# mit-acl/rl_collision_avoidance

Measured on AMD Instinct MI355X. Metric: agent-steps/sec (env.step) at 4 agents x 8192 worlds per GPU, higher is better.
Workload: dtype f64

## Files before the change

### rl_collision_avoidance_amd/csrc/cavoid_capi.hip

```cpp
#include <hip/hip_runtime.h>
#include <hip/hip_ext.h>

#include <cmath>
#include <cstdlib>
#include <cstring>
#include <new>

#include "cavoid.h"
#include "cavoid_host.hpp"
#include "cavoid_kernels.hpp"
#include "cavoid_launch.hpp"
#include "cavoid_crowd.hpp"

using namespace cavoid;

thread_local int g_last_hip_error = 0;

extern "C" int cavoid_abi_version(void) { return CAVOID_ABI_VERSION; }

extern "C" int cavoid_last_hip_error(void) { return g_last_hip_error; }

extern "C" const char *cavoid_strerror(int code) {
    switch (code) {
        case CAVOID_OK: return "ok";
// ... 197 lines not shown
    cold.rvo_collab = cfg->rvo_collab_coeff; cold.rvo_radius_scale = cfg->rvo_radius_scale; cold.rvo_max_dh = cfg->rvo_max_delta_heading;
    cold.gen_min_agents = cfg->gen_min_agents; cold.gen_max_agents = cfg->gen_max_agents;
    KCold *d_cold = reinterpret_cast<KCold *>(static_cast<unsigned char *>(e->slab) + o_act + kActBytes);
    if (hipMemcpy(d_cold, &cold, sizeof(cold), hipMemcpyHostToDevice) != hipSuccess) {
        g_last_hip_error = (int)hipGetLastError();
        cavoid_destroy(e);
        return CAVOID_EHIP;
    }

    KCfg &k = e->k;
    k.cold = d_cold;
    k.dt = cfg->dt;
    k.near_goal_sq = cfg->near_goal_threshold * cfg->near_goal_threshold;
    k.collision_dist = cfg->collision_dist;
    k.close_range = cfg->getting_close_range;
    k.r_goal = cfg->reward_at_goal; k.r_coll = cfg->reward_collision; k.r_close = cfg->reward_getting_close;
    k.r_step = cfg->reward_time_step; k.close_slope = cfg->close_penalty_slope;
    k.clip_lo = cfg->reward_clip_lo; k.clip_hi = cfg->reward_clip_hi;
    k.horizon = cfg->sensing_horizon;
    k.switches = (cfg->done_agents_collide ? 0u : kSwSkipDonePairs) | (cfg->sort_round_gap ? 0u : kSwExactGap) |
                 (cfg->sort_tie_lateral ? 0u : kSwIndexTie) | (cfg->wrap_closed_end ? kSwWrapClosed : 0u);
    k.gen_mode = cfg->gen_mode; k.pool_epoch = cfg->gen_pool_epoch;
    k.rvo_enabled = cfg->rvo_enabled ? 1 : 0;
    k.max_other = cfg->max_other; k.width = 6 + 7 * cfg->max_other;
    k.sort_method = cfg->sort_method; k.dynamics = cfg->dynamics; k.actions_fp32 = cfg->actions_fp32;
    k.timeout_enabled = cfg->timeout_enabled; k.num_actions = cfg->num_actions;
    k.pool_size = cfg->gen_lookahead > 0 ? (int32_t)(e->pool_size > 0x7fffffffLL ? 0x7fffffffLL : e->pool_size) : cfg->gen_pool_size;
    k.ahead = cfg->gen_lookahead;
    k.evaluate_mode = cfg->evaluate_mode ? 1 : 0;
    k.stream_obs = (double)num_worlds * cfg->max_agents * (6 + 7 * cfg->max_other) * sizeof(float) > 16.0 * 1048576.0 ? 1 : 0;
    if (const char *ov = std::getenv("CAVOID_STREAM_OBS")) k.stream_obs = std::atoi(ov) != 0;
    k.seed_lo = 0; k.seed_hi = 0;
    k.num_worlds = num_worlds; k.world_offset = world_offset;
    k.action_table = e->d_actions;

    const int N = cfg->max_agents, wpw_max = 64 / N;
    int wpw = wpw_max;
    if (const char *ov = std::getenv("CAVOID_WPW")) { int v = std::atoi(ov); if (v >= 1 && v <= wpw_max) wpw = v; }
    k.wpw = wpw;
    const int lanes = wpw * N;
    e->latency_mode = (num_worlds * cfg->max_agents <= 64 * 2048 && (cfg->gen_pool_size > 0 || cfg->gen_lookahead > 0)) ? 1 : 0;
    if (const char *ov = std::getenv("CAVOID_PREFETCH_POOL")) {
        const int v = std::atoi(ov);
        e->latency_mode = (v != 0 && (cfg->gen_pool_size > 0 || cfg->gen_lookahead > 0)) ? 1 : 0;
        e->prefetch_single = e->latency_mode;
    }
    k.prefetch_pool = e->latency_mode;
    if (const char *ov = std::getenv("CAVOID_PIPELINE")) e->pipeline = std::atoi(ov);
    if (const char *ov = std::getenv("CAVOID_QUAD")) e->quad = std::atoi(ov);
    if (const char *ov = std::getenv("CAVOID_RELAY_CONSUMERS")) {
        const int v = std::atoi(ov);
        if (v >= 1 && v <= cavoid::kRelayMaxConsumers) e->relay_consumers = v;
    }
    if (crowd_form(N)) {
        k.rvo_lds_floats = 0;
        k.park_floats = 0;
        int rows = (crowd_key_floats(N) / (k.width + 2)) & ~3;
        if (rows < 4) rows = 4;
        if (rows > lanes) rows = lanes;
        if (const char *ov = std::getenv("CAVOID_TILE_ROWS")) { int v = std::atoi(ov); if (v >= 1 && v <= lanes) rows = v; }
        k.tile_rows = rows;
        if ((size_t)(lds_floats_block() + crowd_wave_floats(N, rows, k.width + 2)) * sizeof(float) > 65536) { cavoid_destroy(e); return CAVOID_EUNSUPPORTED; }
        e->waves_per_block = 1;
        e->grid = grid_for(e, num_worlds);
        *out = e;
        return CAVOID_OK;
    }
    k.rvo_lds_floats = cfg->rvo_enabled ? 64 * 2 * (N - 1) * 4 * 2 : 0;
    k.park_floats = ((N >= kParkFromN && !cfg->rvo_enabled) ? 3 * (N - 1) * 64 : 0) + 256;
    if (k.park_floats < lds_floats_scratch()) k.park_floats = lds_floats_scratch();
    static_assert(64 * 2 * 4 * 2 * (kParkFromN - 1) >= 3 * 64 * (kParkFromN - 1) + 256, "reset / observe of an RVO env park keys, gaps and velocities in the idle ORCA scratch");
    const int row_floats = k.width + 2;
    int tile_rows = (int)(9216 / ((size_t)row_floats * sizeof(float))) & ~3;
    if (tile_rows < 4) tile_rows = 4;
    const bool one_pass_fits = (size_t)(lds_floats_block() + lds_floats_fixed(N) + k.rvo_lds_floats + lanes * row_floats + 4) * sizeof(float) <= 65536;
    if (tile_rows > lanes || (e->latency_mode && one_pass_fits)) tile_rows = lanes;
    if (const char *ov = std::getenv("CAVOID_TILE_ROWS")) { int v = std::atoi(ov); if (v >= 1 && v <= lanes) tile_rows = v; }
    auto wave_bytes = [&](int rows) {
        int tile = (rows * row_floats + 3) & ~3;
        if (tile < k.park_floats) tile = k.park_floats;
        return (size_t)(lds_floats_fixed(N) + k.rvo_lds_floats + tile) * sizeof(float);
    };
    while (tile_rows > 4 && wave_bytes(tile_rows) + lds_floats_block() * sizeof(float) > 65536) tile_rows -= 4;
    k.tile_rows = tile_rows;
    const size_t per_wave = wave_bytes(tile_rows);
    int wpb = (int)(((size_t)65536 - lds_floats_block() * sizeof(float)) / per_wave);
    if (wpb < 1) { cavoid_destroy(e); return CAVOID_EUNSUPPORTED; }
    if (wpb > 4) wpb = 4;
    if (const char *ov = std::getenv("CAVOID_WAVES_PER_BLOCK")) { int v = std::atoi(ov); if (v >= 1 && v <= wpb) wpb = v; }
    e->waves_per_block = wpb;
    e->grid = grid_for(e, num_worlds);
    *out = e;
    return CAVOID_OK;
}

extern "C" void cavoid_destroy(cavoid_env *e) {
    if (!e) return;
    if (e->ev0) (void)hipEventDestroy(e->ev0);
    if (e->ev1) (void)hipEventDestroy(e->ev1);
    if (e->slab) (void)hipFree(e->slab);
    if (e->pool_slab) (void)hipFree(e->pool_slab);
    delete e;
}

extern "C" int64_t cavoid_num_worlds(const cavoid_env *e) { return e ? e->W : 0; }
extern "C" int32_t cavoid_obs_width(const cavoid_env *e) { return e ? e->k.width : 0; }
// ... 353 lines not shown
```

### rl_collision_avoidance_amd/csrc/cavoid_launch.hpp

```cpp
#pragma once
#include <hip/hip_runtime.h>
#include <hip/hip_ext.h>

#include <type_traits>

#include "cavoid.h"
#include "cavoid_host.hpp"
#include "cavoid_kernels.hpp"

struct cavoid_env {
    int device = 0;
    int64_t W = 0, A = 0, world_offset = 0;
    cavoid_cfg cfg{};
    cavoid::KCfg k{};
    cavoid::KState st{};
    cavoid::PoolRec *pool = nullptr;
    uint32_t *pool_episode = nullptr;
    int64_t pool_size = 0;
    int ahead_R = 0;
    uint32_t *ahead_hi[2] = {nullptr, nullptr};
    int ahead_cur = 0;
    int ahead_budget = 0;
    bool ahead_primed = false;
    bool ahead_always = false;
    int64_t ahead_refills = 0;
    int relay_topup_nc = -1;
    size_t relay_topup_lds = 0;
    bool relay_topup_fits = false;
    void *slab = nullptr;
    void *pool_slab = nullptr;
    double *d_actions = nullptr;
    int waves_per_block = 4;
    int grid = 0;
    int pipeline = 2;
    int relay_consumers = 3;
    int latency_mode = 0;
    int quad = -1;
    int prefetch_single = 0;
    int last_form = CAVOID_FORM_NONE;
    int last_relay_consumers = 0;
    hipEvent_t ev0 = nullptr, ev1 = nullptr;
};


namespace cavoid {

template <int... Ns>
struct NList {};
#ifdef CAVOID_DEV_ONLY_N
#ifndef CAVOID_DEV_ENV_NS
#define CAVOID_DEV_ENV_NS 4, 10
#endif
#ifndef CAVOID_DEV_RELAY_NS
#define CAVOID_DEV_RELAY_NS 4
#endif
using EnvNs = NList<CAVOID_DEV_ENV_NS>;
using RelayNs = NList<CAVOID_DEV_RELAY_NS>;
using QuadNs = NList<4>;
#else
using EnvNs = NList<1, 2, 3, 4, 5, 6, 7, 8, 9, 10, 11, 12, 13, 14, 15, 16>;
using RelayNs = NList<1, 2, 3, 4, 5, 6>;
using QuadNs = NList<2, 3, 4, 5, 6, 10>;
#endif

#ifdef CAVOID_DEV_CROWD_FROM_N
constexpr int kCrowdFromN = CAVOID_DEV_CROWD_FROM_N;
#else
constexpr int kCrowdFromN = kTileMaxAgents + 1;
#endif
static inline bool crowd_form(int max_agents) { return max_agents >= kCrowdFromN; }

template <int... Ns, class F>
static inline int dispatch_n(int n, NList<Ns...>, F &&f) {
    int rc = CAVOID_EUNSUPPORTED;
    (void)((n == Ns ? (rc = f(std::integral_constant<int, Ns>{}), true) : false) || ...);
    return rc;
}

template <class K, class... Args>
static inline void launch_kernel(K kernel, dim3 grid, dim3 block, size_t lds, hipStream_t s, hipEvent_t ev_start, hipEvent_t ev_stop,
                                 const Args &...args) {
    if (ev_start || ev_stop) hipExtLaunchKernelGGL(kernel, grid, block, lds, s, ev_start, ev_stop, 0, args...);
    else hipLaunchKernelGGL(kernel, grid, block, lds, s, args...);
}

#ifdef CAVOID_TRACE
static inline int set_trace(unsigned long long *dev_ptr) {
    HIP_TRY(hipMemcpyToSymbol(HIP_SYMBOL(g_trace), &dev_ptr, sizeof(dev_ptr)));
// ... 79 lines not shown
```

### rl_collision_avoidance_amd/csrc/cavoid_relay.hip

```cpp
#include "cavoid_launch.hpp"
#include "cavoid_relay.hpp"

using namespace cavoid;

constexpr int kRelayMaxDevices = 64;
template <int N>
static int relay_allow_lds() {
    static bool allowed[kRelayMaxDevices] = {};
    int dev = 0;
    HIP_TRY(hipGetDevice(&dev));
    const bool cached = dev >= 0 && dev < kRelayMaxDevices;
    if (cached && allowed[dev]) return CAVOID_OK;
    if (hipFuncSetAttribute(reinterpret_cast<const void *>(env_relay_kernel<N>), hipFuncAttributeMaxDynamicSharedMemorySize, (int)kRelayLdsLimit) != hipSuccess) {
        (void)hipGetLastError();
        return CAVOID_EUNSUPPORTED;
    }
    if (cached) allowed[dev] = true;
    return CAVOID_OK;
}

struct RelayShape {
    int nc = 0;
    size_t lds = 0;
    bool topup = false;
};
template <int N>
static int relay_shape_n(cavoid_env *e, int tile_floats, bool want_topup, RelayShape &sh) {
    int nc = e->relay_consumers;
    while (nc > 1 && relay_lds_fixed_bytes<N>() + (size_t)nc * tile_floats * sizeof(float) > kRelayLdsLimit) --nc;
    const size_t lds = relay_lds_fixed_bytes<N>() + (size_t)nc * tile_floats * sizeof(float);
    if (lds > kRelayLdsLimit || (nc < 2 && e->relay_consumers >= 2)) return CAVOID_EUNSUPPORTED;
    if (lds > 65536) {
        const int rc_opt = relay_allow_lds<N>();
        if (rc_opt != CAVOID_OK) return rc_opt;
    }
    sh.nc = nc;
    sh.lds = lds;
    sh.topup = false;
    if (want_topup && e->k.gen_mode == 0) {
        if (e->relay_topup_nc != nc || e->relay_topup_lds != lds) {
            int blocks = 0;
            if (hipOccupancyMaxActiveBlocksPerMultiprocessor(&blocks, reinterpret_cast<const void *>(env_relay_kernel<N>), 64 * (4 + nc), lds) != hipSuccess) {
                (void)hipGetLastError();
                blocks = 0;
            }
            e->relay_topup_nc = nc;
            e->relay_topup_lds = lds;
            e->relay_topup_fits = blocks >= 2;
        }
        sh.topup = e->relay_topup_fits;
    }
    return CAVOID_OK;
}
static int relay_shape(cavoid_env *e, const KIO &io, bool want_topup, RelayShape &sh) {
    const KCfg &k = e->k;
    if (k.rvo_enabled || k.pool_size <= 0 || !io.obs || !io.actions || io.cont) return CAVOID_EUNSUPPORTED;
    if (k.switches & kSwSkipDonePairs) return CAVOID_EUNSUPPORTED;
    const int64_t tiles = (e->W + k.wpw - 1) / k.wpw;
    if (tiles > 512) return CAVOID_EUNSUPPORTED;
    if (e->cfg.max_agents > kRelayMaxAgents) return CAVOID_EUNSUPPORTED;
    const int row = io.obs_stride;
    const int tile_floats = (k.tile_rows * row + 3) & ~3;
    if (k.tile_rows < k.wpw * e->cfg.max_agents) return CAVOID_EUNSUPPORTED;
    return dispatch_n(e->cfg.max_agents, RelayNs{}, [&](auto n) -> int { return relay_shape_n<decltype(n)::value>(e, tile_floats, want_topup, sh); });
}

static bool relay_wants_topup(const cavoid_env *e, hipStream_t s) {
    if (e->ahead_R <= 0 || e->ahead_always || e->k.gen_mode != 0) return false;
    hipStreamCaptureStatus cap = hipStreamCaptureStatusNone;
    (void)hipStreamIsCapturing(s, &cap);
    return cap == hipStreamCaptureStatusNone;
}

bool cavoid_relay_takes_topup(cavoid_env *e, const KIO &io, hipStream_t s) {
    RelayShape sh;
    return relay_wants_topup(e, s) && relay_shape(e, io, true, sh) == CAVOID_OK && sh.topup;
}

int cavoid_launch_relay(cavoid_env *e, const KIO &io, hipStream_t s, hipEvent_t ev_start, hipEvent_t ev_stop) {
    RelayShape sh;
    const int rc_shape = relay_shape(e, io, io.ahead_hi != nullptr, sh);
    if (rc_shape != CAVOID_OK) return rc_shape;
    if ((io.ahead_hi != nullptr) != sh.topup) return CAVOID_EINVAL;
    const int64_t tiles = (e->W + e->k.wpw - 1) / e->k.wpw;
    const dim3 grid((unsigned)tiles), block(64 * (3 + sh.nc + (sh.topup ? 1 : 0)));
    const int rc = dispatch_n(e->cfg.max_agents, RelayNs{}, [&](auto n) -> int {
        launch_kernel(env_relay_kernel<decltype(n)::value>, grid, block, sh.lds, s, ev_start, ev_stop, e->k, e->st, e->pool, io);
        return CAVOID_OK;
    });
    if (rc != CAVOID_OK) return rc;
    HIP_TRY(hipGetLastError());
    return note_form(e, CAVOID_OK, CAVOID_FORM_RELAY, sh.nc);
}

#ifdef CAVOID_TRACE
int cavoid_debug_trace_relay(unsigned long long *dev_ptr) { return set_trace(dev_ptr); }
#endif
```

### rl_collision_avoidance_amd/csrc/cavoid_relay.hpp

```cpp
#pragma once
#include <cstddef>
#include <type_traits>

#include "cavoid_kernels.hpp"

namespace cavoid {

constexpr int kRelayMaxAgents = 6;
template <int N>
__host__ __device__ constexpr int relay_ring() { return N <= 5 ? 8 : 4; }
constexpr size_t kRelayLdsLimit = 80 * 1024;
constexpr int kRelayActRing = 64;
constexpr int kRelayActAhead = 48;
constexpr int kRelayEvq = 8;
constexpr int kRelayTopupMaxN = 5;

struct RelaySeq {
    int spec;
    int stage;
    int res;
    int fin;
    int act;
    int ev;
    int nxt;
    int cons[kRelayMaxConsumers];
    int cfin[kRelayMaxConsumers];
    int coop[2];
    int kernarg[2];
    int tile_id;
};
static_assert(sizeof(RelaySeq) % 16 == 0, "the event queue behind it holds 64-bit masks; the tiles further on are read 16 bytes at a time");
struct RelayTent { double px[64], py[64], vx[64], vy[64], heading[64]; float r[64], gx[64], gy[64], pref[64]; uint32_t flags[64]; };
struct RelayRes { uint32_t flags[64], ctl[64]; float rew[64]; };
struct RelayNxt { double px[64], py[64], heading[64], t_rem[64]; float gx[64], gy[64], radius[64], pref[64]; uint32_t flags[64]; };
#ifndef CAVOID_RELAY_ORDER
#define CAVOID_RELAY_ORDER 0x6432150
#endif
#ifndef CAVOID_RELAY_PRIO_D
#define CAVOID_RELAY_PRIO_D 3
#endif
#ifndef CAVOID_RELAY_PRIO_P
#define CAVOID_RELAY_PRIO_P 3
#endif
#ifndef CAVOID_RELAY_PRIO_L
#define CAVOID_RELAY_PRIO_L 0
#endif
#ifndef CAVOID_RELAY_PRIO_C
#define CAVOID_RELAY_PRIO_C 1
#endif
#ifndef CAVOID_RELAY_PRIO_T
#define CAVOID_RELAY_PRIO_T 0
#endif
#ifndef CAVOID_RELAY_ABL
#define CAVOID_RELAY_ABL 0
#endif
__device__ __forceinline__ int relay_role_of(int wv, int NC) {
    if (NC == 3) return (int)(((unsigned)CAVOID_RELAY_ORDER >> (4 * wv)) & 15u);
    return wv;
}
constexpr int kRelayCoopWaves = 3;
constexpr int kRelayCoopFromN = 4;
template <int N>
struct RelayCoop {
    static constexpr int K = Others<N>::K;
    uint64_t key[K][64];
    uint32_t bits[K][64];
};
template <int N>
__host__ __device__ constexpr size_t relay_coop_bytes() { return N >= kRelayCoopFromN ? sizeof(RelayCoop<N>) : 0; }
template <int N>
__host__ __device__ constexpr size_t relay_lds_fixed_bytes() {
    return (size_t)lds_floats_block() * sizeof(float) + sizeof(RelaySeq) + kRelayActRing * 64 + relay_ring<N>() * (sizeof(RelayTent) + sizeof(RelayRes)) +
           sizeof(RelayNxt) + kRelayEvq * sizeof(unsigned long long) + relay_coop_bytes<N>();
}

#ifdef CAVOID_TRACE
#define RELAY_STAMP(k)                                                                                         \
    do {                                                                                                       \
        if (lane0 == 0 && g_trace && t == (n_steps >> 1)) g_trace[wave * 32 + (k)] = (unsigned long long)clock64(); \
    } while (0)
#define RELAY_MARK(k)                                                                                          \
    do {                                                                                                       \
        if (lane0 == 0 && g_trace) g_trace[wave * 32 + (k)] = (unsigned long long)clock64();                   \
    } while (0)
#else
#define RELAY_STAMP(k) do { } while (0)
#define RELAY_MARK(k) do { } while (0)
#endif

typedef __attribute__((address_space(3))) volatile int relay_lds_int;
__device__ __forceinline__ int relay_peek(const int *p) { return __builtin_amdgcn_readfirstlane(*(relay_lds_int *)p); }
__device__ __forceinline__ void relay_wait(const int *p, int v) {
    while (relay_peek(p) < v) __builtin_amdgcn_s_sleep(1);
    asm volatile("" ::: "memory");
}
constexpr int kRelayPollLimit = 1 << 24;
__device__ __forceinline__ void relay_wait_bounded(const int *p, int v) {
    int polls = 0;
    while (relay_peek(p) < v) {
        if (++polls > kRelayPollLimit) __builtin_trap();
        __builtin_amdgcn_s_sleep(1);
    }
    asm volatile("" ::: "memory");
}
__device__ __forceinline__ void relay_spin(const int *p, int v) {
    while (relay_peek(p) < v) { }
    asm volatile("" ::: "memory");
}
__device__ __forceinline__ int relay_peek_issue(const int *p) { return *(relay_lds_int *)p; }
__device__ __forceinline__ int relay_seen(int v) { return __builtin_amdgcn_readfirstlane(v); }
typedef __attribute__((address_space(3))) volatile uint32_t relay_lds_u32;
typedef __attribute__((address_space(3))) volatile double relay_lds_f64;
__device__ __forceinline__ void relay_post(int *p, int v) {
    asm volatile("" ::: "memory");
    *(relay_lds_int *)p = v;
    asm volatile("" ::: "memory");
}

struct RelayTrig {
    double two_over_pi, pio2_hi, pio2_lo, s1, s2, s3, s4, s5, s6, c1, c2, c3, c4, c5, c6;
};
__device__ __forceinline__ RelayTrig relay_trig_constants() {
    RelayTrig k;
    k.two_over_pi = 0.63661977236758134308; k.pio2_hi = 1.57079632673412561417e+00; k.pio2_lo = 6.07710050650619224932e-11;
    k.s6 = 1.58969099521155010221e-10; k.s5 = -2.50507602534068634195e-08; k.s4 = 2.75573137070700676789e-06;
    k.s3 = -1.98412698298579493134e-04; k.s2 = 8.33333333332248946124e-03; k.s1 = -1.66666666666666324348e-01;
    k.c6 = -1.13596475577881948265e-11; k.c5 = 2.08757232129817482790e-09; k.c4 = -2.75573143513906633035e-07;
// ... 143 lines not shown
        co.key[o][lane] = ((uint64_t)hi << 32) | lo;
        co.bits[o][lane] = seen ? 2u : 0u;
        gapf[o] = (float)gap_o;
        neighbour_features(e, (float)e.prll_x, (float)e.prll_y, rx, ry, q, feat[o]);
    }
}

struct RelayArgs { KCfg c; KState s; const PoolRec *pool; KIO io; };
static_assert(alignof(KCfg) == 8 && alignof(KState) == 8 && alignof(KIO) == 8 && alignof(RelayArgs) == 8, "kernel arguments: 8-byte aligned");
static_assert(sizeof(KCfg) % 8 == 0 && sizeof(KState) % 8 == 0 && sizeof(KIO) % 8 == 0, "kernel arguments: whole 8-byte words, no tail padding to skip");
static_assert(offsetof(RelayArgs, c) == 0 && offsetof(RelayArgs, s) == sizeof(KCfg) && offsetof(RelayArgs, pool) == sizeof(KCfg) + sizeof(KState) &&
                  offsetof(RelayArgs, io) == sizeof(KCfg) + sizeof(KState) + sizeof(const PoolRec *) &&
                  sizeof(RelayArgs) == sizeof(KCfg) + sizeof(KState) + sizeof(const PoolRec *) + sizeof(KIO),
              "RelayArgs must be the kernel's argument segment, argument by argument");
static_assert(sizeof(KIO) == 104 && offsetof(KIO, n_steps) == 80 && offsetof(KIO, ahead_hi) == 96, "KIO changed: check what relay_coop_last reads from it");
template <class T>
__device__ __forceinline__ void relay_load_args(T &dst, const __attribute__((address_space(4))) T *src) {
    static_assert(sizeof(T) % 4 == 0, "whole words");
    const __attribute__((address_space(4))) uint32_t *w = (const __attribute__((address_space(4))) uint32_t *)src;
    uint32_t d[sizeof(T) / 4];
#pragma unroll
    for (int k = 0; k < (int)(sizeof(T) / 4); ++k) d[k] = w[k];
    __builtin_memcpy(&dst, d, sizeof(T));
}
#ifndef CAVOID_RELAY_ROLE_ARGS
#define CAVOID_RELAY_ROLE_ARGS 1
#endif
typedef const __attribute__((address_space(4))) RelayArgs *RelayArgP;
#if CAVOID_RELAY_ROLE_ARGS
#define RELAY_ROLE_ARGS_LOAD()                                                                         \
    unsigned long long kp_ = (unsigned long long)__builtin_amdgcn_kernarg_segment_ptr();               \
    asm volatile("" : "+s"(kp_));                                                                      \
    KCfg c; KState s; const PoolRec *pool; KIO io;                                                     \
    relay_load_args(s, &((RelayArgP)kp_)->s); relay_load_args(io, &((RelayArgP)kp_)->io);               \
    relay_load_args(c, &((RelayArgP)kp_)->c); relay_load_args(pool, &((RelayArgP)kp_)->pool);            \
    asm volatile("" : "+s"(c.wpw), "+s"(c.num_worlds))
#define RELAY_ROLE_PIN(...) asm volatile("" : __VA_ARGS__)
#define RELAY_ROLE_STATE(name)                                                                         \
    unsigned long long kps_ = (unsigned long long)__builtin_amdgcn_kernarg_segment_ptr();              \
    asm volatile("" : "+s"(kps_));                                                                     \
    KState name;                                                                                       \
    relay_load_args(name, &((RelayArgP)kps_)->s)
#else
#define RELAY_ROLE_ARGS_LOAD() const KCfg &c = c_; const KState &s = s_; const PoolRec *const pool = pool_; const KIO &io = io_
#define RELAY_ROLE_STATE(name) const KState &name = s_
#define RELAY_ROLE_PIN(...) do { } while (0)
#endif
#define RELAY_ROLE_ARGS()                                                                              \
    RELAY_ROLE_ARGS_LOAD();                                                                            \
    (void)s; (void)pool;                                                                               \
    [[maybe_unused]] const int ostride = io.obs_stride;                                                \
    [[maybe_unused]] const int tile_floats = (c.tile_rows * ostride + 3) & ~3;                         \
    const int wpw = c.wpw, lanes_used = wpw * N;                                                       \
    [[maybe_unused]] const int64_t wave = blockIdx.x;                      \
    const int64_t w0 = wave * wpw;                                                                     \
    const int lw = lane0 / N;                                                                          \
    [[maybe_unused]] const int i0 = lane0 - lw * N;                                                    \
    [[maybe_unused]] const int64_t w = w0 + lw;                                                        \
    [[maybe_unused]] const bool active = lane0 < lanes_used && w < c.num_worlds;                       \
    [[maybe_unused]] const int base0 = lane0 < lanes_used ? lw * N : 0;                                \
    [[maybe_unused]] const int64_t a_idx0 = w * N + i0;                                                \
    [[maybe_unused]] const bool packed = io.packed != 0;                                               \
    [[maybe_unused]] int64_t worlds_here = c.num_worlds - w0;                                          \
    if (worlds_here > wpw) worlds_here = wpw;                                                          \
    if (worlds_here < 0) worlds_here = 0;                                                              \
    [[maybe_unused]] const int n_steps = io.n_steps
template <int N>
__device__ __forceinline__ void relay_coop_last(unsigned char *smem) {
    unsigned char *sp = smem + lds_floats_block() * sizeof(float);
    RelaySeq *seq = reinterpret_cast<RelaySeq *>(sp); sp += sizeof(RelaySeq) + kRelayEvq * sizeof(unsigned long long);
    const unsigned long long kp = (unsigned long long)(uint32_t)relay_peek(&seq->kernarg[0]) | ((unsigned long long)(uint32_t)relay_peek(&seq->kernarg[1]) << 32);
    typedef const __attribute__((address_space(4))) RelayArgs *ArgP;
    const ArgP ka = (ArgP)kp;
    KCfg c;
    KIO io;
    relay_load_args(c, &ka->c);
    relay_load_args(io, &ka->io);
    RelayTent *tents = reinterpret_cast<RelayTent *>(sp); sp += relay_ring<N>() * sizeof(RelayTent) + sizeof(RelayNxt);
    RelayRes *ress = reinterpret_cast<RelayRes *>(sp); sp += relay_ring<N>() * sizeof(RelayRes) + kRelayActRing * 64;
    RelayCoop<N> *coopb = reinterpret_cast<RelayCoop<N> *>(sp); sp += relay_coop_bytes<N>();
    float *tiles = reinterpret_cast<float *>(sp);
    const int lane0 = threadIdx.x & 63;
    const int tile_nc = relay_peek(&seq->tile_id);
    const int NC = tile_nc >> 16;
    const int role = relay_role_of(threadIdx.x >> 6, NC);
    const int pw = role < 2 ? role : 2;
    const int ostride = io.obs_stride;
    const int tile_floats = (c.tile_rows * ostride + 3) & ~3;
    const int wpw = c.wpw, lanes_used = wpw * N;
    const int64_t wave = tile_nc & 0xFFFF;
    const int64_t w0 = wave * wpw;
    const int lw = lane0 / N, i0 = lane0 - lw * N;
    const int64_t w = w0 + lw;
    const bool active = lane0 < lanes_used && w < c.num_worlds;
    const int base0 = lane0 < lanes_used ? lw * N : 0;
    const int64_t a_idx0 = w * N + i0;
    const bool packed = io.packed != 0;
    int64_t worlds_here = c.num_worlds - w0;
    if (worlds_here > wpw) worlds_here = wpw;
    if (worlds_here < 0) worlds_here = 0;
    const int n_steps = io.n_steps;
    constexpr int K = Others<N>::K;
    const int t = n_steps - 1;
    const int cid_l = t % NC;
    float *tile = tiles + (size_t)cid_l * tile_floats;
    RelayCoop<N> &co = *coopb;
    relay_wait_bounded(&seq->fin, t + 1);
    const RelayTent &f = tents[t & (relay_ring<N>() - 1)];
    const RelayRes &v = ress[t & (relay_ring<N>() - 1)];
    Agent ao;
    ao.px = f.px[lane0]; ao.py = f.py[lane0]; ao.vx = f.vx[lane0]; ao.vy = f.vy[lane0];
    ao.heading = f.heading[lane0]; ao.t_rem = 0.0;
    ao.gx = f.gx[lane0]; ao.gy = f.gy[lane0]; ao.speed = 0.0f;
    ao.radius = f.r[lane0]; ao.pref = f.pref[lane0]; ao.flags = v.flags[lane0];
    const uint32_t ctl_c = v.ctl[lane0];
    const float rew_c = v.rew[lane0], done_c = (ctl_c & 1u) ? 1.0f : 0.0f;
    const bool present = active && (ao.flags & CAVOID_F_PRESENT);
    const Ego e = ego_frame_obs(c, ao);
    const ArrayStage<N> as{f.px, f.py, f.vx, f.vy, f.r, i0, base0};
    float gapf[K], feat[K][kFeat];
#pragma unroll
    for (int o = 0; o < K; ++o) {
        gapf[o] = 0.0f;
#pragma unroll
        for (int q = 0; q < kFeat; ++q) feat[o][q] = 0.0f;
    }
    if (c.switches != 0u) relay_pair_part<N, true>(c, ao, e, present, as, pw, lane0, co, gapf, feat);
    else relay_pair_part<N, false>(c, ao, e, present, as, pw, lane0, co, gapf, feat);
    relay_coop_arrive(&seq->coop[0], lane0);
    Key key[K];
    uint32_t valid = 0u;
    if (N == 1) key[0].set(kKeySentinel, 0u);
#pragma unroll
    for (int o = 0; o < N - 1; ++o) {
        key[o].v = co.key[o][lane0];
        valid |= (co.bits[o][lane0] & 2u) ? (1u << o) : 0u;
    }
    if (t - NC >= 0) relay_wait_bounded(&seq->cons[cid_l], t - NC + 1);
    const int rows_active = (int)worlds_here * N;
    assemble_obs<N, false, true, ArrayStage<N>, NoHook, false, PartOthers>(c, ao, e, active, lane0, as, key, gapf, feat, valid, tile, nullptr,
                                                                           rows_active, ostride, false, 0.0f, 0.0f, wave, NoHook(), false, nullptr,
                                                                           PartOthers{pw, kRelayCoopWaves});
    if (pw == 0 && active && lane0 < rows_active) {
        const int M = c.max_other;
        const int m = __popc(valid);
        const int first = m > M ? m - M : 0;
        const int kept = m - first;
        write_row_head(tile + lane0 * ostride, ao, e, present, kept, kept, M, packed, c.width, rew_c, done_c);
    }
    relay_coop_arrive(&seq->coop[1], lane0);
    if (io.out_step_stride == 0)
        for (int o = 0; o < NC; ++o) relay_wait_bounded(&seq->cfin[o], 1);
    const int64_t slot_w = (int64_t)t * io.out_step_stride;
    if (worlds_here > 0) {
        float *dst = io.obs + (slot_w + w0) * N * ostride;
        const bool lines = ((rows_active * ostride) & 31) == 0 && (reinterpret_cast<uintptr_t>(dst) & 127) == 0;
        if (io.out_step_stride != 0 && lines) flush_tile<4, true, true>(tile, dst, rows_active * ostride, pw * 64 + lane0, 64 * kRelayCoopWaves);
        else if (io.out_step_stride != 0) flush_tile<4, true>(tile, dst, rows_active * ostride, pw * 64 + lane0, 64 * kRelayCoopWaves);
        else flush_tile<4>(tile, dst, rows_active * ostride, pw * 64 + lane0, 64 * kRelayCoopWaves);
    }
    if (pw == 0 && active) {
        if (!packed) {
            io.rew[slot_w * N + a_idx0] = rew_c;
            io.done[slot_w * N + a_idx0] = (ctl_c & 1u) ? 1 : 0;
        }
        if (i0 == 0) io.game_over[slot_w + w] = (ctl_c & 2u) ? 1 : 0;
    }
    if (pw == 0) RELAY_MARK(29);
}

template <int N>
__device__ __forceinline__ void relay_topup() {
    __builtin_amdgcn_s_setprio(CAVOID_RELAY_PRIO_T);
    unsigned long long kp = (unsigned long long)__builtin_amdgcn_kernarg_segment_ptr();
    asm volatile("" : "+s"(kp));
    typedef const __attribute__((address_space(4))) RelayArgs *ArgP;
    const ArgP ka = (ArgP)kp;
    KCfg c;
    uint32_t *episode, *hi;
    const PoolRec *ring;
    relay_load_args(c, &ka->c);
    relay_load_args(episode, &ka->s.episode);
    relay_load_args(ring, &ka->pool);
    relay_load_args(hi, &ka->io.ahead_hi);
    const int lane0 = threadIdx.x & 63;
    const int wpw = c.wpw, lanes_used = wpw * N;
    const int lw = lane0 / N, i0 = lane0 - lw * N;
    const int64_t w = (int64_t)blockIdx.x * wpw + lw;
    const bool active = lane0 < lanes_used && w < c.num_worlds;
    const int base0 = lane0 < lanes_used ? lw * N : 0;
    uint32_t ep = 0u, fh = 0u;
    if (active) {
        ep = episode[w];
        fh = hi[w];
    }
    asm volatile("" : "+v"(ep), "+v"(fh));
    __syncthreads();
    ahead_fill_range<N, true>(c, ep, fh, active, w, i0, base0, lane0, hi, const_cast<PoolRec *>(ring), c.ahead, 0, 1, nullptr, nullptr);
}

template <int N>
__global__ void __launch_bounds__(64 * (4 + kRelayMaxConsumers), N <= kRelayTopupMaxN ? 4 : 1) env_relay_kernel(const KCfg c_, const KState s_, const PoolRec *pool_, const KIO io_) {
    extern __shared__ __attribute__((aligned(16))) unsigned char smem[];
    unsigned char *sp = smem;
    double *lds_tab = reinterpret_cast<double *>(sp); sp += lds_floats_block() * sizeof(float);
    RelaySeq *seq = reinterpret_cast<RelaySeq *>(sp); sp += sizeof(RelaySeq);
    unsigned long long *evq = reinterpret_cast<unsigned long long *>(sp); sp += kRelayEvq * sizeof(unsigned long long);
    RelayTent *tents = reinterpret_cast<RelayTent *>(sp); sp += relay_ring<N>() * sizeof(RelayTent);
    RelayNxt *nbuf = reinterpret_cast<RelayNxt *>(sp); sp += sizeof(RelayNxt);
    RelayRes *ress = reinterpret_cast<RelayRes *>(sp); sp += relay_ring<N>() * sizeof(RelayRes);
    unsigned char *actring = sp; sp += kRelayActRing * 64;
    RelayCoop<N> *coopb = reinterpret_cast<RelayCoop<N> *>(sp); sp += relay_coop_bytes<N>();
    float *tiles = reinterpret_cast<float *>(sp);

    const int NC = (blockDim.x >> 6) - 3 - (io_.ahead_hi ? 1 : 0);
    const int role = relay_role_of(threadIdx.x >> 6, NC);
    const int lane0 = threadIdx.x & 63;
    constexpr bool kCoop = N >= kRelayCoopFromN;
    const bool coop_role = role < 2 || role == 2 + NC;

    if (role == 0 && lane0 < (int)(sizeof(RelaySeq) / sizeof(int))) reinterpret_cast<int *>(seq)[lane0] = 0;
    if constexpr (kCoop) {
        if (role == 0 && lane0 == 0) {
            const unsigned long long kp = (unsigned long long)__builtin_amdgcn_kernarg_segment_ptr();
            seq->kernarg[0] = (int)(uint32_t)kp; seq->kernarg[1] = (int)(uint32_t)(kp >> 32);
            seq->tile_id = (int)blockIdx.x | (NC << 16);
        }
    }

    if (role == 0) {
        __builtin_amdgcn_s_setprio(CAVOID_RELAY_PRIO_D);
        RELAY_ROLE_ARGS();
        RELAY_ROLE_PIN("+s"(s.px), "+s"(s.py), "+s"(s.heading), "+s"(s.t_rem), "+s"(s.gx), "+s"(s.gy), "+s"(s.radius), "+s"(s.pref), "+s"(s.flags),
                       "+s"(s.episode), "+s"(io.actions), "+s"(c.action_table));
        RELAY_MARK(20);
        KCfg cd = c;
        asm volatile("" : "+s"(cd.dt), "+s"(cd.near_goal_sq), "+s"(cd.actions_fp32), "+s"(cd.dynamics),
                     "+s"(cd.timeout_enabled), "+s"(cd.switches));
        const RelayTrig trig = relay_trig_constants();
        Agent a;
        a.px = a.py = a.heading = a.t_rem = a.vx = a.vy = 0.0;
        a.gx = a.gy = a.radius = a.pref = a.speed = 0.0f;
        a.flags = 0u;
        uint32_t episode = 0u;
        double tab_v = 0.0;
        if (lane0 < 2 * c.num_actions) tab_v = c.action_table[lane0];
        int act0 = 0;
        if (active) {
            episode = s.episode[w];
            load_agent(s, a_idx0, a);
            act0 = io.actions[a_idx0];
        }
        if (cd.actions_fp32 && (lane0 & 1)) tab_v = (double)(float)tab_v;
        lds_tab[lane0] = tab_v;
        act0 = act0 < 0 ? 0 : (act0 >= c.num_actions ? c.num_actions - 1 : act0);
        const bool present_first = active && (a.flags & CAVOID_F_PRESENT);
        bool restarted_any = false, moved_any = false;
        int events = 0;
        bool T_moving;
        Agent T;
        wave_lds_sync();
        RelayStatics ks = relay_statics(a, active);
        T = relay_advance(cd, trig, a, ks, lds_tab[2 * act0], lds_tab[2 * act0 + 1], active, T_moving);
        __syncthreads();
        RELAY_MARK(21);
        double tab_s = 0.0, tab_h = 0.0;
        int act_q = 0;
        if (n_steps > 1) {
            const int actn = (int)actring[64 + lane0];
            tab_s = lds_tab[2 * actn]; tab_h = lds_tab[2 * actn + 1];
            if (n_steps > 2) act_q = (int)actring[2 * 64 + lane0];
        }
        auto stage_out = [&](RelayTent &tn, const Agent &x, float r_staged, int lane) {
            tn.px[lane] = x.px; tn.py[lane] = x.py; tn.r[lane] = r_staged; tn.flags[lane] = x.flags;
            tn.vx[lane] = x.vx; tn.vy[lane] = x.vy; tn.heading[lane] = x.heading;
            tn.gx[lane] = x.gx; tn.gy[lane] = x.gy; tn.pref[lane] = x.pref;
        };
        stage_out(tents[0], T, ks.r_staged, lane0);
        relay_post(&seq->spec, 1);
// ... 214 lines not shown
                }
                loaded = loaded + 8 < upto ? loaded + 8 : upto;
            }
        };
        load_actions(n_steps < 8 ? n_steps : 8);
        RELAY_MARK(26);
        __syncthreads();
        relay_post(&seq->act, loaded);
        {
            Agent r0;
            absent_agent(r0);
            if (active) load_pool(pool, (int64_t)pool_index(c, (uint32_t)(c.world_offset + w), ep + 1u) * N + i0, r0);
            RelayNxt &nb = *nbuf;
            nb.px[lane0] = r0.px; nb.py[lane0] = r0.py; nb.heading[lane0] = r0.heading; nb.t_rem[lane0] = r0.t_rem;
            nb.gx[lane0] = r0.gx; nb.gy[lane0] = r0.gy; nb.radius[lane0] = r0.radius; nb.pref[lane0] = r0.pref;
            nb.flags[lane0] = r0.flags;
            relay_post(&seq->nxt, 1);
            RELAY_MARK(27);
        }
        int served = 0, idle_polls = 0;
        while (true) {
            const int ev = relay_peek(&seq->ev), fin = relay_peek(&seq->fin);
            if (served < ev) {
                asm volatile("" ::: "memory");
                const unsigned long long mask = evq[served & (kRelayEvq - 1)];
                if ((mask >> lane0) & 1ull) {
                    ep += 1u;
                    Agent r0;
                    load_pool(pool, (int64_t)pool_index(c, (uint32_t)(c.world_offset + w), ep + 1u) * N + i0, r0);
                    RelayNxt &nb = *nbuf;
                    nb.px[lane0] = r0.px; nb.py[lane0] = r0.py; nb.heading[lane0] = r0.heading; nb.t_rem[lane0] = r0.t_rem;
                    nb.gx[lane0] = r0.gx; nb.gy[lane0] = r0.gy; nb.radius[lane0] = r0.radius; nb.pref[lane0] = r0.pref;
                    nb.flags[lane0] = r0.flags;
                }
                served += 1;
                idle_polls = 0;
                relay_post(&seq->nxt, served + 1);
                continue;
            }
            if (loaded < n_steps && loaded < fin + kRelayActAhead) {
                int upto = fin + kRelayActAhead;
                if (upto > loaded + 8) upto = loaded + 8;
                if (upto > n_steps) upto = n_steps;
                load_actions(upto);
                idle_polls = 0;
                relay_post(&seq->act, loaded);
                continue;
            }
            if (fin >= n_steps && relay_peek(&seq->stage) > n_steps) break;
            if (++idle_polls > kRelayPollLimit) __builtin_trap();
            __builtin_amdgcn_s_sleep(2);
        }
    } else if (role == 3 + NC) {
        relay_topup<N>();
    } else {
        __builtin_amdgcn_s_setprio(CAVOID_RELAY_PRIO_C);
        RELAY_ROLE_ARGS();
        KCfg cc = c;
        asm volatile("" : "+s"(cc.switches));
        const int cid = role - 2;
        float *tile = tiles + (size_t)cid * tile_floats;
        __syncthreads();
        const int n_mine = kCoop ? n_steps - 1 : n_steps;
        for (int t = cid; t < n_mine; t += NC) {
            int lane = lane0, i = i0, base = base0;
            asm volatile("" : "+v"(lane), "+v"(i), "+v"(base));
            RELAY_STAMP(16);
            relay_wait_bounded(&seq->fin, t + 1);
            RELAY_STAMP(17);
            if (CAVOID_RELAY_ABL & 1) { relay_post(&seq->cons[cid], t + 1); continue; }
            const RelayTent &f = tents[t & (relay_ring<N>() - 1)];
            const RelayRes &v = ress[t & (relay_ring<N>() - 1)];
            Agent ao;
            ao.px = f.px[lane]; ao.py = f.py[lane]; ao.vx = f.vx[lane]; ao.vy = f.vy[lane];
            ao.heading = f.heading[lane]; ao.t_rem = 0.0;
            ao.gx = f.gx[lane]; ao.gy = f.gy[lane]; ao.speed = 0.0f;
            ao.radius = f.r[lane]; ao.pref = f.pref[lane]; ao.flags = v.flags[lane];
            const uint32_t ctl_c = v.ctl[lane];
            const float rew_c = v.rew[lane], done_c = (ctl_c & 1u) ? 1.0f : 0.0f;
            const bool present = active && (ao.flags & CAVOID_F_PRESENT);
            const Ego e = ego_frame_obs(cc, ao);
            Key key[Others<N>::K];
            float gapf[Others<N>::K];
            uint32_t valid;
            bool hit;
            double min_gap;
            const ArrayStage<N> as{f.px, f.py, f.vx, f.vy, f.r, i, base};
            float feat[Others<N>::K][kFeat];
            pair_pass<N, false, true>(cc, ao, e, present, as, key, gapf, feat, valid, hit, min_gap);
            RELAY_STAMP(18);
            const bool last = t == n_steps - 1 && io.out_step_stride == 0;
            const int64_t slot_w = (int64_t)t * io.out_step_stride;
            auto order_last = [&]() {
                if (last)
                    for (int o = 0; o < NC; ++o)
                        if (o != cid) relay_wait_bounded(&seq->cfin[o], 1);
            };
            assemble_obs<N, false, true, ArrayStage<N>, decltype(order_last)>(cc, ao, e, active, lane, as, key, gapf, feat, valid, tile,
                                         io.obs + (slot_w + w0) * N * ostride, (int)worlds_here * N, ostride, packed, rew_c, done_c, wave,
                                         order_last, io.out_step_stride != 0);
            if (active) {
                if (!packed) {
                    io.rew[slot_w * N + a_idx0] = rew_c;
                    io.done[slot_w * N + a_idx0] = (ctl_c & 1u) ? 1 : 0;
                }
                if (i0 == 0) io.game_over[slot_w + w] = (ctl_c & 2u) ? 1 : 0;
            }
            relay_post(&seq->cons[cid], t + 1);
            RELAY_STAMP(19);
            if (t == 0) RELAY_MARK(28);
            if (t == n_steps - 1) RELAY_MARK(29);
        }
        __builtin_amdgcn_s_waitcnt(0);
        if (cid == 0) RELAY_MARK(30);
        relay_post(&seq->cfin[cid], 1);
    }
    if constexpr (kCoop) {
        if (coop_role) relay_coop_last<N>(smem);
    }
}
static_assert(std::is_same<decltype(&env_relay_kernel<4>), void (*)(const KCfg, const KState, const PoolRec *, const KIO)>::value,
              "relay_coop_last reloads the kernel's arguments through RelayArgs: keep the two in step");

}
```

Baseline: 25.03 billion.

## Pack two relay tiles per workgroup with interleaved wave roles

Adds a TPW=2 variant of the relay kernel in which one workgroup hosts two independent tiles. Each has its own LDS region, and the waves of the two tiles are interleaved by a slot map. For N=4, it is chosen by default when the tile count is at least twice the CU count, and the default consumer count rises to 4 in that mode. The aim is better packing of relay pipelines per CU and less per-workgroup launch overhead. The cost is a larger LDS footprint, launch bounds of 1024 threads, and an occupancy check that may fall back to one tile per workgroup.

```diff
diff --git a/rl_collision_avoidance_amd/csrc/cavoid_capi.hip b/rl_collision_avoidance_amd/csrc/cavoid_capi.hip
--- a/rl_collision_avoidance_amd/csrc/cavoid_capi.hip
+++ b/rl_collision_avoidance_amd/csrc/cavoid_capi.hip
@@ -273,6 +273,10 @@
         const int v = std::atoi(ov);
         if (v >= 1 && v <= cavoid::kRelayMaxConsumers) e->relay_consumers = v;
     }
+    if (const char *ov = std::getenv("CAVOID_RELAY_TILES")) {
+        const int v = std::atoi(ov);
+        if (v == 1 || v == 2) e->relay_tiles = v;
+    }
     if (crowd_form(N)) {
         k.rvo_lds_floats = 0;
         k.park_floats = 0;
diff --git a/rl_collision_avoidance_amd/csrc/cavoid_launch.hpp b/rl_collision_avoidance_amd/csrc/cavoid_launch.hpp
--- a/rl_collision_avoidance_amd/csrc/cavoid_launch.hpp
+++ b/rl_collision_avoidance_amd/csrc/cavoid_launch.hpp
@@ -27,13 +27,18 @@
     int relay_topup_nc = -1;
     size_t relay_topup_lds = 0;
     bool relay_topup_fits = false;
+    int relay_tiles = 0;
+    int relay_duo_nc = -1;
+    size_t relay_duo_lds = 0;
+    int relay_duo_fit = 0;
+    int relay_cus = 0;
     void *slab = nullptr;
     void *pool_slab = nullptr;
     double *d_actions = nullptr;
     int waves_per_block = 4;
     int grid = 0;
     int pipeline = 2;
-    int relay_consumers = 3;
+    int relay_consumers = 0;
     int latency_mode = 0;
     int quad = -1;
     int prefetch_single = 0;
diff --git a/rl_collision_avoidance_amd/csrc/cavoid_relay.hip b/rl_collision_avoidance_amd/csrc/cavoid_relay.hip
--- a/rl_collision_avoidance_amd/csrc/cavoid_relay.hip
+++ b/rl_collision_avoidance_amd/csrc/cavoid_relay.hip
@@ -4,14 +4,15 @@
 using namespace cavoid;
 
 constexpr int kRelayMaxDevices = 64;
-template <int N>
+constexpr int kRelaySoloConsumers = 3, kRelayDuoConsumers = 4;
+template <int N, int TPW = 1>
 static int relay_allow_lds() {
     static bool allowed[kRelayMaxDevices] = {};
     int dev = 0;
     HIP_TRY(hipGetDevice(&dev));
     const bool cached = dev >= 0 && dev < kRelayMaxDevices;
     if (cached && allowed[dev]) return CAVOID_OK;
-    if (hipFuncSetAttribute(reinterpret_cast<const void *>(env_relay_kernel<N>), hipFuncAttributeMaxDynamicSharedMemorySize, (int)kRelayLdsLimit) != hipSuccess) {
+    if (hipFuncSetAttribute(reinterpret_cast<const void *>(env_relay_kernel<N, TPW>), hipFuncAttributeMaxDynamicSharedMemorySize, (int)(TPW * kRelayLdsLimit)) != hipSuccess) {
         (void)hipGetLastError();
         return CAVOID_EUNSUPPORTED;
     }
@@ -23,20 +24,83 @@
     int nc = 0;
     size_t lds = 0;
     bool topup = false;
+    int tpw = 1;
 };
+static bool relay_duo_wanted(cavoid_env *e, int n, int64_t tiles) {
+    if (n > kRelayDuoMaxN || e->relay_tiles == 1) return false;
+    if (e->relay_tiles == 2) return true;
+    if (n != 4) return false;
+    if (e->relay_cus <= 0) {
+        int dev = 0, cus = 0;
+        if (hipGetDevice(&dev) != hipSuccess || hipDeviceGetAttribute(&cus, hipDeviceAttributeMultiprocessorCount, dev) != hipSuccess || cus <= 0) {
+            (void)hipGetLastError();
+            return false;
+        }
+        e->relay_cus = cus;
+    }
+    return (tiles + 1) / 2 >= e->relay_cus;
+}
+template <int N>
+static bool relay_duo_fits(cavoid_env *e, int nc, size_t lds, bool want_topup, bool &topup) {
+    if constexpr (N > kRelayDuoMaxN) return false;
+    else {
+        if (e->relay_duo_nc != nc || e->relay_duo_lds != lds) {
+            e->relay_duo_nc = nc;
+            e->relay_duo_lds = lds;
+            e->relay_duo_fit = 0;
+            const void *fn = reinterpret_cast<const void *>(env_relay_kernel<N, 2>);
+            hipFuncAttributes fa{};
+            int lim = 0, dev = 0;
+            bool ok = hipGetDevice(&dev) == hipSuccess && hipFuncGetAttributes(&fa, fn) == hipSuccess && fa.localSizeBytes == 0 &&
+                      hipDeviceGetAttribute(&lim, hipDeviceAttributeMaxSharedMemoryPerBlock, dev) == hipSuccess;
+            if (ok && lds > (size_t)lim) {
+                int optin = 0;
+                if (hipDeviceGetAttribute(&optin, hipDeviceAttributeSharedMemPerBlockOptin, dev) == hipSuccess && optin > 0) ok = lds <= (size_t)optin;
+            }
+            ok = ok && (lds <= 65536 || relay_allow_lds<N, 2>() == CAVOID_OK);
+            for (int t = 1; ok && t >= 0; --t) {
+                int blocks = 0;
+                if (hipOccupancyMaxActiveBlocksPerMultiprocessor(&blocks, fn, 64 * relay_duo_waves(nc, t), lds) == hipSuccess && blocks >= 1) e->relay_duo_fit |= 1 << t;
+            }
+            (void)hipGetLastError();
+        }
+        topup = want_topup && (e->relay_duo_fit & 2) != 0;
+        return (e->relay_duo_fit & (topup ? 2 : 1)) != 0;
+    }
+}
 template <int N>
 static int relay_shape_n(cavoid_env *e, int tile_floats, bool want_topup, RelayShape &sh) {
-    int nc = e->relay_consumers;
-    while (nc > 1 && relay_lds_fixed_bytes<N>() + (size_t)nc * tile_floats * sizeof(float) > kRelayLdsLimit) --nc;
-    const size_t lds = relay_lds_fixed_bytes<N>() + (size_t)nc * tile_floats * sizeof(float);
-    if (lds > kRelayLdsLimit || (nc < 2 && e->relay_consumers >= 2)) return CAVOID_EUNSUPPORTED;
+    auto consumers = [&](int dflt, int &asked) {
+        int nc = asked = e->relay_consumers > 0 ? e->relay_consumers : dflt;
+        while (nc > 1 && relay_region_bytes(relay_lds_fixed_bytes<N>(), nc, tile_floats) > kRelayLdsLimit) --nc;
+        return nc;
+    };
+    sh.topup = false;
+    const int64_t tiles = (e->W + e->k.wpw - 1) / e->k.wpw;
+    if (relay_duo_wanted(e, N, tiles)) {
+        int asked = 0;
+        const int nc2 = consumers(kRelayDuoConsumers, asked);
+        const size_t lds2 = relay_lds_bytes(2, relay_lds_fixed_bytes<N>(), nc2, tile_floats);
+        bool topup2 = false;
+        if (lds2 <= 2 * kRelayLdsLimit && !(nc2 < 2 && asked >= 2) && relay_duo_fits<N>(e, nc2, lds2, want_topup && e->k.gen_mode == 0, topup2)) {
+            sh.nc = nc2;
+            sh.lds = lds2;
+            sh.topup = topup2;
+            sh.tpw = 2;
+            return CAVOID_OK;
+        }
+    }
+    int asked = 0;
+    const int nc = consumers(kRelaySoloConsumers, asked);
+    const size_t lds = relay_region_bytes(relay_lds_fixed_bytes<N>(), nc, tile_floats);
+    if (lds > kRelayLdsLimit || (nc < 2 && asked >= 2)) return CAVOID_EUNSUPPORTED;
     if (lds > 65536) {
         const int rc_opt = relay_allow_lds<N>();
         if (rc_opt != CAVOID_OK) return rc_opt;
     }
     sh.nc = nc;
     sh.lds = lds;
-    sh.topup = false;
+    sh.tpw = 1;
     if (want_topup && e->k.gen_mode == 0) {
         if (e->relay_topup_nc != nc || e->relay_topup_lds != lds) {
             int blocks = 0;
@@ -72,6 +136,8 @@
     return cap == hipStreamCaptureStatusNone;
 }
 
+static int g_relay_last_tiles = 0;
+
 bool cavoid_relay_takes_topup(cavoid_env *e, const KIO &io, hipStream_t s) {
     RelayShape sh;
     return relay_wants_topup(e, s) && relay_shape(e, io, true, sh) == CAVOID_OK && sh.topup;
@@ -83,14 +149,38 @@
     if (rc_shape != CAVOID_OK) return rc_shape;
     if ((io.ahead_hi != nullptr) != sh.topup) return CAVOID_EINVAL;
     const int64_t tiles = (e->W + e->k.wpw - 1) / e->k.wpw;
-    const dim3 grid((unsigned)tiles), block(64 * (3 + sh.nc + (sh.topup ? 1 : 0)));
+    const dim3 grid((unsigned)((tiles + sh.tpw - 1) / sh.tpw)), block(64 * sh.tpw * (3 + sh.nc + (sh.topup ? 1 : 0)));
     const int rc = dispatch_n(e->cfg.max_agents, RelayNs{}, [&](auto n) -> int {
-        launch_kernel(env_relay_kernel<decltype(n)::value>, grid, block, sh.lds, s, ev_start, ev_stop, e->k, e->st, e->pool, io);
+        constexpr int N = decltype(n)::value;
+        if constexpr (N <= kRelayDuoMaxN) {
+            if (sh.tpw == 2) {
+                launch_kernel(env_relay_kernel<N, 2>, grid, block, sh.lds, s, ev_start, ev_stop, e->k, e->st, e->pool, io);
+                return CAVOID_OK;
+            }
+        }
+        launch_kernel(env_relay_kernel<N>, grid, block, sh.lds, s, ev_start, ev_stop, e->k, e->st, e->pool, io);
         return CAVOID_OK;
     });
     if (rc != CAVOID_OK) return rc;
     HIP_TRY(hipGetLastError());
+    g_relay_last_tiles = sh.tpw;
     return note_form(e, CAVOID_OK, CAVOID_FORM_RELAY, sh.nc);
+}
+
+extern "C" int32_t cavoid_relay_duo_slot(int32_t wv, int32_t nc, int32_t topup, int32_t mate) {
+    if (wv < 0 || nc < 1 || nc > kRelayMaxConsumers || wv >= relay_duo_waves(nc, topup)) return -1;
+    return relay_duo_slot(wv, nc, mate < 0 ? CAVOID_RELAY_DUO_MATE : mate);
+}
+extern "C" int32_t cavoid_relay_last_tiles(void) { return g_relay_last_tiles; }
+extern "C" int64_t cavoid_relay_lds_layout(int32_t n, int32_t tpw, int32_t nc, int32_t tile_floats, int32_t what) {
+    int64_t r = -1;
+    (void)dispatch_n(n, NList<1, 2, 3, 4, 5, 6>{}, [&](auto nn) -> int {
+        const size_t fixed = relay_lds_fixed_bytes<decltype(nn)::value>();
+        r = what == 2 ? (int64_t)relay_lds_bytes(tpw, fixed, nc, tile_floats) : what == 3 ? (int64_t)relay_region_bytes(fixed, nc, tile_floats)
+                                                                                          : (int64_t)relay_region_offset(what, fixed, nc, tile_floats);
+        return CAVOID_OK;
+    });
+    return r;
 }
 
 #ifdef CAVOID_TRACE
diff --git a/rl_collision_avoidance_amd/csrc/cavoid_relay.hpp b/rl_collision_avoidance_amd/csrc/cavoid_relay.hpp
--- a/rl_collision_avoidance_amd/csrc/cavoid_relay.hpp
+++ b/rl_collision_avoidance_amd/csrc/cavoid_relay.hpp
@@ -73,6 +73,21 @@
     return (size_t)lds_floats_block() * sizeof(float) + sizeof(RelaySeq) + kRelayActRing * 64 + relay_ring<N>() * (sizeof(RelayTent) + sizeof(RelayRes)) +
            sizeof(RelayNxt) + kRelayEvq * sizeof(unsigned long long) + relay_coop_bytes<N>();
 }
+
+#ifndef CAVOID_RELAY_DUO_MATE
+#define CAVOID_RELAY_DUO_MATE 0
+#endif
+constexpr int kRelayDuoMaxN = 5;
+__host__ __device__ constexpr int relay_duo_waves(int NC, int topup) { return 2 * (3 + NC + (topup ? 1 : 0)); }
+__host__ __device__ constexpr int relay_duo_slot(int wv, int NC, int mate = CAVOID_RELAY_DUO_MATE) {
+    if (wv < 4) return ((wv & 1) << 4) | (wv >> 1);
+    const int k = wv - 4;
+    if (k < 2 * NC) return ((((k & 1) ^ mate) & 1) << 4) | (2 + (k >> 1));
+    return (((k - 2 * NC) & 1) << 4) | (2 + NC + ((k - 2 * NC) >> 1));
+}
+__host__ __device__ constexpr size_t relay_region_bytes(size_t fixed, int nc, int tile_floats) { return fixed + (size_t)nc * tile_floats * sizeof(float); }
+__host__ __device__ constexpr size_t relay_lds_bytes(int tpw, size_t fixed, int nc, int tile_floats) { return tpw * relay_region_bytes(fixed, nc, tile_floats); }
+__host__ __device__ constexpr size_t relay_region_offset(int tsel, size_t fixed, int nc, int tile_floats) { return tsel * relay_region_bytes(fixed, nc, tile_floats); }
 
 #ifdef CAVOID_TRACE
 #define RELAY_STAMP(k)                                                                                         \
@@ -322,7 +337,7 @@
     [[maybe_unused]] const int ostride = io.obs_stride;                                                \
     [[maybe_unused]] const int tile_floats = (c.tile_rows * ostride + 3) & ~3;                         \
     const int wpw = c.wpw, lanes_used = wpw * N;                                                       \
-    [[maybe_unused]] const int64_t wave = blockIdx.x;                      \
+    [[maybe_unused]] const int64_t wave = tile_index;       \
     const int64_t w0 = wave * wpw;                                                                     \
     const int lw = lane0 / N;                                                                          \
     [[maybe_unused]] const int i0 = lane0 - lw * N;                                                    \
@@ -335,7 +350,7 @@
     if (worlds_here > wpw) worlds_here = wpw;                                                          \
     if (worlds_here < 0) worlds_here = 0;                                                              \
     [[maybe_unused]] const int n_steps = io.n_steps
-template <int N>
+template <int N, int TPW>
 __device__ __forceinline__ void relay_coop_last(unsigned char *smem) {
     unsigned char *sp = smem + lds_floats_block() * sizeof(float);
     RelaySeq *seq = reinterpret_cast<RelaySeq *>(sp); sp += sizeof(RelaySeq) + kRelayEvq * sizeof(unsigned long long);
@@ -353,8 +368,14 @@
     const int lane0 = threadIdx.x & 63;
     const int tile_nc = relay_peek(&seq->tile_id);
     const int NC = tile_nc >> 16;
-    const int role = relay_role_of(threadIdx.x >> 6, NC);
-    const int pw = role < 2 ? role : 2;
+    int pw;
+    if constexpr (TPW == 2) {
+        const int wv = (int)(threadIdx.x >> 6);
+        pw = wv < 2 ? 0 : (wv < 4 ? 1 : 2);
+    } else {
+        const int role = relay_role_of(threadIdx.x >> 6, NC);
+        pw = role < 2 ? role : 2;
+    }
     const int ostride = io.obs_stride;
     const int tile_floats = (c.tile_rows * ostride + 3) & ~3;
     const int wpw = c.wpw, lanes_used = wpw * N;
@@ -440,7 +461,7 @@
 }
 
 template <int N>
-__device__ __forceinline__ void relay_topup() {
+__device__ __forceinline__ void relay_topup(const unsigned tile_index) {
     __builtin_amdgcn_s_setprio(CAVOID_RELAY_PRIO_T);
     unsigned long long kp = (unsigned long long)__builtin_amdgcn_kernarg_segment_ptr();
     asm volatile("" : "+s"(kp));
@@ -456,7 +477,7 @@
     const int lane0 = threadIdx.x & 63;
     const int wpw = c.wpw, lanes_used = wpw * N;
     const int lw = lane0 / N, i0 = lane0 - lw * N;
-    const int64_t w = (int64_t)blockIdx.x * wpw + lw;
+    const int64_t w = (int64_t)tile_index * wpw + lw;
     const bool active = lane0 < lanes_used && w < c.num_worlds;
     const int base0 = lane0 < lanes_used ? lw * N : 0;
     uint32_t ep = 0u, fh = 0u;
@@ -469,9 +490,28 @@
     ahead_fill_range<N, true>(c, ep, fh, active, w, i0, base0, lane0, hi, const_cast<PoolRec *>(ring), c.ahead, 0, 1, nullptr, nullptr);
 }
 
-template <int N>
-__global__ void __launch_bounds__(64 * (4 + kRelayMaxConsumers), N <= kRelayTopupMaxN ? 4 : 1) env_relay_kernel(const KCfg c_, const KState s_, const PoolRec *pool_, const KIO io_) {
-    extern __shared__ __attribute__((aligned(16))) unsigned char smem[];
+template <int N, int TPW = 1>
+__global__ void __launch_bounds__(TPW == 2 ? 1024 : 64 * (4 + kRelayMaxConsumers), TPW == 2 ? 1 : (N <= kRelayTopupMaxN ? 4 : 1)) env_relay_kernel(const KCfg c_, const KState s_, const PoolRec *pool_, const KIO io_) {
+    static_assert(TPW == 1 || TPW == 2, "one or two tiles per workgroup");
+    static_assert(relay_lds_fixed_bytes<N>() % 16 == 0, "a tile's region begins on a 16-byte boundary (TPW = 2: the second one behind the first)");
+    extern __shared__ __attribute__((aligned(16))) unsigned char smem_wg[];
+    const int NC = (blockDim.x >> (TPW == 2 ? 7 : 6)) - 3 - (io_.ahead_hi ? 1 : 0);
+    int role;
+    unsigned tile_index;
+    unsigned char *smem = smem_wg;
+    if constexpr (TPW == 2) {
+        const int slot = relay_duo_slot(__builtin_amdgcn_readfirstlane((int)(threadIdx.x >> 6)), NC);
+        role = slot & 15;
+        tile_index = 2u * blockIdx.x + (unsigned)(slot >> 4);
+        smem += relay_region_offset(slot >> 4, relay_lds_fixed_bytes<N>(), NC, (c_.tile_rows * io_.obs_stride + 3) & ~3);
+        if ((int64_t)tile_index * c_.wpw >= c_.num_worlds) {
+            __syncthreads();
+            return;
+        }
+    } else {
+        role = relay_role_of(threadIdx.x >> 6, NC);
+        tile_index = blockIdx.x;
+    }
     unsigned char *sp = smem;
     double *lds_tab = reinterpret_cast<double *>(sp); sp += lds_floats_block() * sizeof(float);
     RelaySeq *seq = reinterpret_cast<RelaySeq *>(sp); sp += sizeof(RelaySeq);
@@ -483,8 +523,6 @@
     RelayCoop<N> *coopb = reinterpret_cast<RelayCoop<N> *>(sp); sp += relay_coop_bytes<N>();
     float *tiles = reinterpret_cast<float *>(sp);
 
-    const int NC = (blockDim.x >> 6) - 3 - (io_.ahead_hi ? 1 : 0);
-    const int role = relay_role_of(threadIdx.x >> 6, NC);
     const int lane0 = threadIdx.x & 63;
     constexpr bool kCoop = N >= kRelayCoopFromN;
     const bool coop_role = role < 2 || role == 2 + NC;
@@ -494,7 +532,7 @@
         if (role == 0 && lane0 == 0) {
             const unsigned long long kp = (unsigned long long)__builtin_amdgcn_kernarg_segment_ptr();
             seq->kernarg[0] = (int)(uint32_t)kp; seq->kernarg[1] = (int)(uint32_t)(kp >> 32);
-            seq->tile_id = (int)blockIdx.x | (NC << 16);
+            seq->tile_id = (int)tile_index | (NC << 16);
         }
     }
 
@@ -815,7 +853,7 @@
             __builtin_amdgcn_s_sleep(2);
         }
     } else if (role == 3 + NC) {
-        relay_topup<N>();
+        relay_topup<N>(tile_index);
     } else {
         __builtin_amdgcn_s_setprio(CAVOID_RELAY_PRIO_C);
         RELAY_ROLE_ARGS();
@@ -879,7 +917,7 @@
         relay_post(&seq->cfin[cid], 1);
     }
     if constexpr (kCoop) {
-        if (coop_role) relay_coop_last<N>(smem);
+        if (coop_role) relay_coop_last<N, TPW>(smem);
     }
 }
 static_assert(std::is_same<decltype(&env_relay_kernel<4>), void (*)(const KCfg, const KState, const PoolRec *, const KIO)>::value,
```

New measurement: 27.55 billion (median of 6 runs). 1.1x the previous value.
